# linum-uqam/ViT-OCM-WMSegmentation

Measured on AMD Instinct MI355X. Metric: OCM tiles/s (224x224, ViT-S/16 attention-map inference), higher is better.
Workload: dtype bf16x3

## Files before the change

vit-ocm-wmsegmentation_amd/csrc/dev_knobs.h:

```cpp
#pragma once
#ifdef OCM_DEV
extern int g_ocm_knobs[8];
#define OCM_KNOB(i) (g_ocm_knobs[(i)])
#else
#define OCM_KNOB(i) 0
#endif
```

vit-ocm-wmsegmentation_amd/csrc/engine.hip:

```cpp
#include <stdarg.h>
#include <stdio.h>
#include <string.h>

#include <atomic>
#include <mutex>
#include <string>
#include <vector>

#include "host_common.h"
#include "launch.h"
#include "dev_knobs.h"
#include "attn_plan.h"
#include "otsu.h"

static thread_local std::string g_err;

int ocm_fail(int code, const char *fmt, ...) {
    char buf[512];
    va_list ap;
    va_start(ap, fmt);
    vsnprintf(buf, sizeof buf, fmt, ap);
    va_end(ap);
    g_err = buf;
    return code;
}
#define fail ocm_fail

Prof g_prof;

extern "C" int ocm_prof_begin(uint32_t class_mask, int32_t max_launches) {
    std::lock_guard<std::mutex> lk(g_prof.mu);
    if (g_prof.on.load(std::memory_order_relaxed)) return fail(OCM_ESTATE, "profiling already active");
    if (max_launches <= 0) return fail(OCM_EINVAL, "max_launches must be positive");
    g_prof.ev.resize((size_t)max_launches * 2);
    g_prof.cls.assign(max_launches, 0);
    for (auto &e : g_prof.ev) HIP_TRY(hipEventCreate(&e));
    g_prof.used = 0;
    g_prof.mask = class_mask;
    ++g_prof.gen;
    g_prof.on.store(true, std::memory_order_release);
    return OCM_OK;
}

extern "C" int ocm_prof_end(double *ms_per_class, int64_t *launches_per_class) {
    std::lock_guard<std::mutex> lk(g_prof.mu);
    if (!g_prof.on.load(std::memory_order_relaxed)) return fail(OCM_ESTATE, "profiling is not active");
    g_prof.on.store(false, std::memory_order_release);
    for (int c = 0; c < OCM_K_COUNT; ++c) {
        if (ms_per_class) ms_per_class[c] = 0.0;
        if (launches_per_class) launches_per_class[c] = 0;
    }
    int rc = OCM_OK;
    for (size_t i = 0; i < g_prof.used; ++i) {
        float ms = 0.f;
        hipError_t e = hipEventSynchronize(g_prof.ev[2 * i + 1]);
        if (e == hipSuccess) e = hipEventElapsedTime(&ms, g_prof.ev[2 * i], g_prof.ev[2 * i + 1]);
        if (e != hipSuccess) {
            rc = fail(OCM_EHIP, "event timing failed: %s", hipGetErrorString(e));
            break;
        }
        if (ms_per_class) ms_per_class[g_prof.cls[i]] += ms;
        if (launches_per_class) launches_per_class[g_prof.cls[i]] += 1;
    }
    for (auto &e : g_prof.ev) (void)hipEventDestroy(e);
    g_prof.ev.clear();
    g_prof.cls.clear();
    g_prof.used = 0;
    return rc;
}

#ifdef OCM_DEV
extern "C" int ocm_debug_knob(int32_t which, int32_t value) {
    if (which < 0 || which >= 8) return fail(OCM_EINVAL, "knob %d out of range", which);
    g_ocm_knobs[which] = value;
    return OCM_OK;
}
#endif

extern "C" int ocm_abi_version(void) { return OCM_ABI_VERSION; }
extern "C" const char *ocm_last_error(void) { return g_err.c_str(); }
extern "C" int32_t ocm_n_pad(int32_t n_tokens) { return ocm_round_up(n_tokens, 8); }
extern "C" int32_t ocm_n_pad_prec(int32_t precision, int32_t n_tokens) { return ocm_n_pad_for(precision, n_tokens); }

enum ParamKind { P_F32, P_BF16, P_PATCH };
struct Param {
    std::string name;
    ParamKind kind;
    size_t count;
    size_t offset;
    bool set;
    bool optional = false;
};

struct BlockP {
    int ln1_g, ln1_b, qkv_w, qkv_b, proj_w, proj_b, ln2_g, ln2_b, fc1_w, fc1_b, fc2_w, fc2_b;
    int qkv_w32 = -1, fc1_w32 = -1, qkv_wf = -1, fc1_wf = -1, qkv_c = -1, qkv_d = -1, fc1_c = -1, fc1_d = -1;
    bool fold_dirty = true;
};

struct ocm_vit {
    ocm_vit_config cfg;
    int D, H, L, M, p, C, Kpe;
    int hd;
    bool mfma_heads() const { return hd == 64 || hd == 128; }
    int prec;
    size_t esz;
    std::vector<Param> params;
    std::vector<BlockP> blk;
    int cls, pe_w, pe_b, norm_g, norm_b, mask_tok;
    char *arena;
    size_t arena_bytes;
    hipGraphExec_t graph_exec = nullptr;
    hipStream_t graph_stream = nullptr;
    ocm_vit_io graph_key;
    bool graph_valid = false;
    uint64_t graph_hits = 0, graph_captures = 0;
    int32_t opt[OCM_OPT_COUNT] = {0};
    bool can_fold() const { return prec == 2; }
    bool folding() const { return can_fold() && opt[OCM_OPT_FOLD_LN] != 1; }

    int add(const std::string &name, ParamKind kind, size_t count, size_t stored_elems) {
        Param pr{name, kind, count, arena_bytes, false};
        const size_t bytes = stored_elems * (kind == P_F32 ? 4 : esz);
        arena_bytes += (bytes + 255) & ~(size_t)255;
        params.push_back(pr);
        return (int)params.size() - 1;
// ... 918 lines not shown
```

vit-ocm-wmsegmentation_amd/csrc/gemm_core.h:

```cpp
#pragma once
#include <type_traits>
#include "common.h"

#ifdef OCM_GEMM_STAMPS
__device__ unsigned long long g_wstamps[512 * 16 * 8];
#define WSTAMP(k)                                                                                       \
    do {                                                                                                \
        if (t == nsteps / 2 && (threadIdx.x & 63) == 0 && blockIdx.x < 512)                              \
            g_wstamps[(blockIdx.x * 16 + (threadIdx.x >> 6 & 15)) * 8 + (k)] = __builtin_readcyclecounter(); \
    } while (0)
__device__ unsigned long long g_stamps[8192 * 8];
#define STAMP(i)                                                                                        \
    do {                                                                                                \
        if (threadIdx.x == 0 && blockIdx.x < 8192) g_stamps[blockIdx.x * 8 + (i)] = __builtin_readcyclecounter(); \
    } while (0)
#else
#define STAMP(i) ((void)0)
#define WSTAMP(k) ((void)0)
#endif

template <int BM_, int BN_, int WAVES_M_, int WAVES_N_, int MF16_ = 0>
struct GemmCfg {
    static constexpr int BM = BM_, BN = BN_, WAVES_M = WAVES_M_, WAVES_N = WAVES_N_, MF16 = MF16_;
    static constexpr int NT = WAVES_M * WAVES_N * OCM_WAVE;
// ... 443 lines not shown
    int bc = 0, bi = D % NSTAGE;
#ifdef OCM_GEMM_STAMPS
    unsigned long long stamp_wait = 0;
#endif
    for (int t = 0; t < nsteps; ++t) {
        const int younger = min(D - 1, nsteps - 1 - t);
#ifdef OCM_GEMM_STAMPS
        const unsigned long long tw0 = __builtin_readcyclecounter();
#endif
        WSTAMP(0);
        wait_vm_steps<LPS, NSTAGE - 2>(younger);
        WSTAMP(1);
#ifdef OCM_GEMM_STAMPS
        const unsigned long long tw1 = __builtin_readcyclecounter();
#endif
        raw_barrier();
#ifdef OCM_GEMM_STAMPS
        if (t == 0) STAMP(6);
        if (t > 0) {
            const unsigned long long tw2 = __builtin_readcyclecounter();
            stamp_wait += ((tw2 - tw1) << 32) | ((tw1 - tw0) & 0xFFFFFFFFull);
        }
#endif
        WSTAMP(2);
#if !defined(OCM_ABL) || OCM_ABL != 2
        if (t + D < nsteps) OCM_DMA_ISSUE(t + D, bi);
#endif
        __builtin_amdgcn_sched_barrier(0);
        WSTAMP(3);
        compute(bc);
#ifdef OCM_GEMM_STAMPS
        if (t == nsteps / 2) {
            __builtin_amdgcn_sched_barrier(0);
            asm volatile("v_mov_b32 %0, %0\n\ts_nop 0" : "+v"(acc[TM - 1][TN - 1][15]));
            WSTAMP(4);
        }
#endif
        bc = bc + 1 == NSTAGE ? 0 : bc + 1;
        bi = bi + 1 == NSTAGE ? 0 : bi + 1;
    }
    raw_barrier();
#ifdef OCM_GEMM_STAMPS
    if (threadIdx.x == 0 && blockIdx.x < 8192) g_stamps[blockIdx.x * 8 + 7] = stamp_wait;
#endif
#undef OCM_DMA_ISSUE
}

constexpr int EPI_MAXS = 6;
struct EpiPre {
    f32x2 raw[EPI_MAXS];
    f32x2 cd;
};
struct EpiNoPre {};
template <class Cfg, class Epi>
__device__ __forceinline__ auto epi_prefetch(const Epi &epi, int m0, int n0, int M, int N) {
    if constexpr (Epi::ROWTAB) {
        EpiPre p;
#pragma unroll
        for (int i = 0; i < EPI_MAXS; ++i) p.raw[i] = f32x2{0.f, 0.f};
        p.cd = f32x2{0.f, 0.f};
        if (threadIdx.x < Cfg::BM) epi.row_raw(min(m0 + (int)threadIdx.x, M - 1), p.raw);
        if (threadIdx.x < Cfg::BN) p.cd = epi.col_entry(min(n0 + (int)threadIdx.x, N - 1));
        return p;
    } else {
        return EpiNoPre();
    }
}

template <class Cfg, bool SWAP, class Epi, int LDS_AVAIL = Cfg::LDS_BYTES, class Pre = EpiNoPre, int ACCL = 0>
__device__ __forceinline__ void run_epilogue(const f32x16 (&acc)[Cfg::TM][Cfg::TN], char *smem, const Epi &epi, int m0,
                                             int n0, bool active = true, const Pre *pre = nullptr) {
    f32x2 *rowtab = (f32x2 *)(smem + LDS_AVAIL), *coltab = rowtab + Cfg::BM;
    if constexpr (Epi::ROWTAB) {
        if (threadIdx.x < Cfg::BM) rowtab[threadIdx.x] = epi.row_final(pre->raw);
        if (threadIdx.x < Cfg::BN) coltab[threadIdx.x] = pre->cd;
    }
    const int lane = threadIdx.x & 63, wave = threadIdx.x >> 6;
    const int wm = wave / Cfg::WAVES_N, wn = wave % Cfg::WAVES_N;
    const int r = lane & 31, h = lane >> 5;
    if constexpr (Cfg::BM * Cfg::BN * 4 <= LDS_AVAIL) {
        constexpr int COLS = SWAP ? Cfg::BM : Cfg::BN;
        float *C = (float *)smem;
        if (active)
#pragma unroll
        for (int i = 0; i < Cfg::TM; ++i)
#pragma unroll
            for (int j = 0; j < Cfg::TN; ++j) {
                const bool half = Cfg::HALF && i == Cfg::TM - 1;
                const int tm = half ? (Cfg::TM - 1) * Cfg::RB + wm * 16 : (i * Cfg::WAVES_M + wm) * 32, tn = (j * Cfg::WAVES_N + wn) * 32;
                const int row0 = SWAP ? tn : tm, col0 = SWAP ? tm : tn;
#pragma unroll
                for (int e = 0; e < (half ? 8 : 16); ++e)
                    C[(row0 + acc_rpos<ACCL>(e, lane)) * COLS + col0 + acc_cpos<ACCL>(e, lane)] = acc[i][j][e];
            }
        STAMP(2);
        lds_barrier();
        STAMP(3);
        if (active) epi.template run<PassCfg<Cfg::BM, Cfg::BN, Cfg::NT>>((const float *)C, m0, n0, rowtab, coltab);
    } else if constexpr (!SWAP) {
        constexpr int PASS = Cfg::RB * Cfg::BN * 4;
        static_assert(PASS <= LDS_AVAIL, "a row band must fit the operand LDS");
        constexpr int NBUF = 2 * PASS <= LDS_AVAIL ? 2 : 1;
#pragma unroll
        for (int i = 0; i < Cfg::TM; ++i) {
            if (NBUF == 1 && i) lds_barrier();
            float *C = (float *)(smem + (i % NBUF) * PASS);
            const bool half = Cfg::HALF && i == Cfg::TM - 1;
            if (active)
#pragma unroll
            for (int j = 0; j < Cfg::TN; ++j) {
                const int col0 = (j * Cfg::WAVES_N + wn) * 32;
#pragma unroll
                for (int e = 0; e < (half ? 8 : 16); ++e)
                    C[(wm * (half ? 16 : 32) + acc_rpos<ACCL>(e, lane)) * Cfg::BN + col0 + acc_cpos<ACCL>(e, lane)] = acc[i][j][e];
            }
            lds_barrier();
            if (active) {
                if (half)
                    epi.template run<PassCfg<Cfg::RB / 2, Cfg::BN, Cfg::NT>>((const float *)C, m0 + i * Cfg::RB, n0, rowtab + i * Cfg::RB, coltab);
                else
                    epi.template run<PassCfg<Cfg::RB, Cfg::BN, Cfg::NT>>((const float *)C, m0 + i * Cfg::RB, n0, rowtab + i * Cfg::RB, coltab);
            }
        }
    } else {
        static_assert(!Cfg::HALF, "half tiles: normal orientation only");
        constexpr int PASS = Cfg::CB * Cfg::BM * 4;
        static_assert(PASS <= LDS_AVAIL, "a column band must fit the operand LDS");
        constexpr int NBUF = 2 * PASS <= LDS_AVAIL ? 2 : 1;
#pragma unroll
        for (int j = 0; j < Cfg::TN; ++j) {
            if (NBUF == 1 && j) lds_barrier();
            float *C = (float *)(smem + (j % NBUF) * PASS);
            if (active)
#pragma unroll
            for (int i = 0; i < Cfg::TM; ++i) {
                const int col0 = (i * Cfg::WAVES_M + wm) * 32;
#pragma unroll
                for (int e = 0; e < 16; ++e)
                    C[(wn * 32 + acc_rpos<ACCL>(e, lane)) * Cfg::BM + col0 + acc_cpos<ACCL>(e, lane)] = acc[i][j][e];
            }
            lds_barrier();
            if (active) epi.template run<PassCfg<Cfg::BM, Cfg::CB, Cfg::NT>>((const float *)C, m0, n0 + j * Cfg::CB, rowtab, coltab + j * Cfg::CB);
        }
    }
}

template <class Cfg, class E, bool SWAP, int KSTEPS, int NSTAGE, class Epi, int A_AUX = 0>
__global__ __launch_bounds__(Cfg::NT) void gemm_dma_kernel(const E *__restrict__ A, int64_t lda, const E *__restrict__ W,
                                                           int64_t ldw, int M, int N, int K, Epi epi) {
    extern __shared__ __attribute__((aligned(16))) char smem[];
    const int tiles_n = (N + Cfg::BN - 1) / Cfg::BN;
    const int id = xcd_remap(blockIdx.x, gridDim.x);
    const int tm = id / tiles_n, tn = id - tm * tiles_n;
    const int m0 = tm * Cfg::BM, n0 = tn * Cfg::BN;
    f32x16 acc[Cfg::TM][Cfg::TN];
    const auto pre = epi_prefetch<Cfg>(epi, m0, n0, M, N);
    STAMP(0);
#if defined(OCM_ABL) && OCM_ABL == 4
#pragma unroll
    for (int i = 0; i < Cfg::TM; ++i)
#pragma unroll
        for (int j = 0; j < Cfg::TN; ++j)
#pragma unroll
            for (int e = 0; e < 16; ++e) acc[i][j][e] = (float)(threadIdx.x + e);
#else
    gemm_mainloop_dma<Cfg, E, SWAP, KSTEPS, NSTAGE, A_AUX>(A, lda, W, ldw, m0, n0, M, N, K, smem, acc, epi.bias);
#endif
    STAMP(1);
#if defined(OCM_ABL) && OCM_ABL == 3
#pragma unroll
    for (int i = 0; i < Cfg::TM; ++i)
#pragma unroll
        for (int j = 0; j < Cfg::TN; ++j) asm volatile("" ::"v"(acc[i][j]));
#else
    run_epilogue<Cfg, SWAP, Epi, NSTAGE * (Cfg::BM + Cfg::BN) * 128, decltype(pre), accl_of<Cfg, E>()>(acc, smem, epi, m0, n0, true, &pre);
#endif
    STAMP(4);
#ifdef OCM_GEMM_STAMPS
    __builtin_amdgcn_s_waitcnt(0);
    STAMP(5);
#endif
}

template <class Cfg, class E, bool SWAP, int KSTEPS, class ALoad, class Epi>
__global__ __launch_bounds__(Cfg::NT) void gemm_kernel(ALoad al, const E *__restrict__ W, int64_t ldw, int M, int N,
                                                       int K, Epi epi) {
    extern __shared__ __attribute__((aligned(16))) char smem[];
    const int tiles_n = (N + Cfg::BN - 1) / Cfg::BN;
    const int id = xcd_remap(blockIdx.x, gridDim.x);
    const int tm = id / tiles_n, tn = id - tm * tiles_n;
    const int m0 = tm * Cfg::BM, n0 = tn * Cfg::BN;
    f32x16 acc[Cfg::TM][Cfg::TN];
    const auto pre = epi_prefetch<Cfg>(epi, m0, n0, M, N);
    STAMP(0);
    gemm_mainloop<Cfg, E, SWAP, KSTEPS>(al, W, ldw, m0, n0, M, N, K, smem, acc, epi.bias);
    STAMP(1);
    run_epilogue<Cfg, SWAP, Epi, Cfg::LDS_BYTES, decltype(pre), accl_of<Cfg, E>()>(acc, smem, epi, m0, n0, true, &pre);
    STAMP(4);
#ifdef OCM_GEMM_STAMPS
    __builtin_amdgcn_s_waitcnt(0);
    STAMP(5);
#endif
}
```

vit-ocm-wmsegmentation_amd/csrc/gemm_kernels.h:

```cpp
#pragma once
#include <type_traits>
#include "gemm_core.h"
#include "launch.h"
#include "gemm_plan.h"
#include "dev_knobs.h"

int ocm_wt_mask();

template <GemmTile T>
using CfgOf = GemmCfg<GEMM_TILES[T].bm, GEMM_TILES[T].bn, GEMM_TILES[T].waves_m, GEMM_TILES[T].waves_n, GEMM_TILES[T].mf16>;
typedef CfgOf<T128x128> Cfg128x128;
typedef CfgOf<T128x128q> Cfg128x128q;
typedef CfgOf<T128x128q16> Cfg128x128q16;
typedef CfgOf<T128x128m16> Cfg128x128m16;
typedef CfgOf<T160x128q16> Cfg160x128q16;
typedef CfgOf<T256x256m16> Cfg256x256m16;
typedef CfgOf<T64x128> Cfg64x128;
typedef CfgOf<T64x128w> Cfg64x128w;
typedef CfgOf<T64x64> Cfg64x64;
typedef CfgOf<T256x256> Cfg256x256;
typedef CfgOf<T256x128> Cfg256x128;
typedef CfgOf<T128x192> Cfg128x192;
typedef CfgOf<T128x96> Cfg128x96;

// ... 94 lines not shown
            const int q = threadIdx.x + i * NT, row = q / CPR, col = (q - row * CPR) * W;
            const int m = m0 + row, n = n0 + col;
            if ((TOTAL % NT != 0 && q >= TOTAL) || m >= M || n >= N) continue;
            const int64_t o = (int64_t)m * ldo + n;
            f32x4 v0 = *(const f32x4 *)(C + row * BN + col);
            if (!ACT_OUT) {
                if (MODE == 1) v0 += rs[i];
                if (MODE == 4) {
#pragma unroll
                    for (int e = 0; e < 4; ++e) v0[e] = fmaxf(v0[e], 0.f);
                }
                *(f32x4 *)((float *)out + o) = v0;
            } else {
                f32x4 v1 = v0;
                if (W == 8) v1 = *(const f32x4 *)(C + row * BN + col + 4);
                if (ln.stats) {
                    const f32x2 mr = rowtab[row];
                    const float mu = mr[0], rstd = mr[1];
#pragma unroll
                    for (int e = 0; e < 4; ++e) {
                        const f32x2 cd = coltab[col + e];
                        v0[e] = fmaf(rstd, fmaf(-mu, cd[0], v0[e]), cd[1]);
                    }
                    if (W == 8) {
#pragma unroll
                        for (int e = 0; e < 4; ++e) {
                            const f32x2 cd = coltab[col + 4 + e];
                            v1[e] = fmaf(rstd, fmaf(-mu, cd[0], v1[e]), cd[1]);
                        }
                    }
                }
                if (MODE == 2) {
#pragma unroll
                    for (int e = 0; e < 4; e += 2) {
                        const f32x2 a = gelu_erf2(f32x2{v0[e], v0[e + 1]});
                        v0[e] = a[0];
                        v0[e + 1] = a[1];
                        if (W == 8) {
                            const f32x2 b = gelu_erf2(f32x2{v1[e], v1[e + 1]});
                            v1[e] = b[0];
                            v1[e + 1] = b[1];
                        }
                    }
                }
                if (wt)
                    store_act_wt((OE *)nullptr, (char *)out + (int64_t)m * ldo * (int)sizeof(OE), n, v0, v1);
                else
                    store_act((OE *)nullptr, (char *)out + (int64_t)m * ldo * (int)sizeof(OE), n, v0, v1);
            }
        }
    }
};

template <class OE>
struct EpiResidStats {
    static constexpr bool ROWTAB = false;
    static constexpr int BN_MULT = 64;
    const float *bias;
    const float *resid;
    float *x;
    void *xs;
    float *stats;
    int M, N;
    int wt = 3;
    float *shift = nullptr;
    const float *prev_stats = nullptr, *prev_shift = nullptr;
    __device__ __forceinline__ static void st16(void *p, const f32x4 &v, bool through) {
        if (through)
            asm volatile("global_store_dwordx4 %0, %1, off sc1\n\ts_nop 1" ::"v"(p), "v"(v) : "memory");
        else
            *(f32x4 *)p = v;
    }
    template <class Cfg>
    __device__ __forceinline__ void run(const float *C, int m0, int n0, const f32x2 *, const f32x2 *) const {
        constexpr int BM = Cfg::BM, BN = Cfg::BN, NT = Cfg::NT, NV = BN / 64, RPP = NT / 8;
        static_assert(BN % 64 == 0 && NT % 64 == 0, "eight lanes x eight columns per chunk");
        const int sub = threadIdx.x & 7, grp = threadIdx.x >> 3;
        constexpr int NPASS = (BM + RPP - 1) / RPP, NPRE = NPASS <= 2 ? NPASS : 1;
        f32x4 pre[NPRE][NV][2];
#pragma unroll
        for (int ps = 0; ps < NPRE; ++ps) {
            const int64_t mo = (int64_t)min(m0 + ps * RPP + grp, M - 1) * N;
#pragma unroll
            for (int i = 0; i < NV; ++i) {
                pre[ps][i][0] = *(const f32x4 *)(resid + mo + n0 + sub * 8 + i * 64);
                pre[ps][i][1] = *(const f32x4 *)(resid + mo + n0 + sub * 8 + i * 64 + 4);
            }
        }
#pragma unroll 2
        for (int r0 = 0; r0 < BM; r0 += RPP) {
            const int row = r0 + grp, m = m0 + row;
            const bool ok = row < BM && m < M;
            const int64_t mo = (int64_t)min(m, M - 1) * N;
            f32x4 v[NV][2];
#pragma unroll
            for (int i = 0; i < NV; ++i) {
                if (NPRE == NPASS) {
                    v[i][0] = pre[NPASS == 2 && r0 ? 1 : 0][i][0];
                    v[i][1] = pre[NPASS == 2 && r0 ? 1 : 0][i][1];
                } else {
                    v[i][0] = *(const f32x4 *)(resid + mo + n0 + sub * 8 + i * 64);
                    v[i][1] = *(const f32x4 *)(resid + mo + n0 + sub * 8 + i * 64 + 4);
                }
            }
            float sh = 0.f;
            if (shift) {
                const int nslot = N >> 6;
                float ps = 0.f;
                if (prev_stats)
                    for (int i = sub; i < nslot; i += 8) ps += prev_stats[((int64_t)min(m, M - 1) * nslot + i) * 2];
#pragma unroll
                for (int o = 4; o > 0; o >>= 1) ps += __shfl_xor(ps, o, 64);
                sh = (prev_shift ? prev_shift[min(m, M - 1)] : 0.f) + ps / (float)N;
                if (ok && n0 == 0 && sub == 0) shift[m] = sh;
            }
            float s1 = 0.f, s2 = 0.f;
            char *rowp = (char *)xs + mo * (int)sizeof(OE);
#pragma unroll
            for (int i = 0; i < NV; ++i) {
                const int n = n0 + sub * 8 + i * 64;
                const float *cp = C + min(row, BM - 1) * BN + sub * 8 + i * 64;
                v[i][0] += *(const f32x4 *)cp;
                v[i][1] += *(const f32x4 *)(cp + 4);
                if (ok) {
                    st16(x + mo + n, v[i][0], wt & 1);
                    st16(x + mo + n + 4, v[i][1], wt & 1);
                }
                v[i][0] -= sh;
                v[i][1] -= sh;
                if (ok) {
                    if constexpr (Elem<OE>::MODE == 2) {
                        bf16x8 hi, lo;
                        split8(v[i][0], v[i][1], hi, lo);
                        st16(rowp + sp_off(n), __builtin_bit_cast(f32x4, hi), wt & 2);
                        st16(rowp + sp_off(n) + 64, __builtin_bit_cast(f32x4, lo), wt & 2);
                    } else if constexpr (Elem<OE>::MODE == 1) {
                        *(f32x4 *)(rowp + n * 4) = v[i][0];
                        *(f32x4 *)(rowp + n * 4 + 16) = v[i][1];
                    } else {
                        *(bf16x8 *)(rowp + n * 2) = cvt8(v[i][0], v[i][1]);
                    }
                }
#pragma unroll
                for (int e = 0; e < 4; ++e) {
                    s1 += v[i][0][e] + v[i][1][e];
                    s2 = fmaf(v[i][0][e], v[i][0][e], fmaf(v[i][1][e], v[i][1][e], s2));
                }
            }
#pragma unroll
            for (int o = 4; o > 0; o >>= 1) {
                s1 += __shfl_xor(s1, o, 64);
                s2 += __shfl_xor(s2, o, 64);
            }
            if (ok && sub < NV) {
                const f32x2 val = {sub ? 0.f : s1, sub ? 0.f : s2};
                *((f32x2 *)stats + (int64_t)m * (N >> 6) + (n0 >> 6) + sub) = val;
            }
        }
    }
};

template <class Cfg, class E, bool SWAP, int KSTEPS, class ALoad, class Epi>
static hipError_t launch_gemm_ks(const ALoad &al, const E *w, int64_t ldw, int M, int N, int K, const Epi &epi,
                                 hipStream_t s) {
    auto kern = gemm_kernel<Cfg, E, SWAP, KSTEPS, ALoad, Epi>;
    constexpr int LDS = Cfg::LDS_BYTES + (Epi::ROWTAB ? (Cfg::BM + Cfg::BN) * 8 : 0);
// ... 127 lines not shown
                                hipStream_t s) {
    EpiLinear<4, E> epi{bias, nullptr, out, M, N, ldo};
    return launch_linear_epi<4, E>(a, w, epi, M, N, K, s);
}

template <class Cfg, class E, int KSTEPS, int NSTAGE>
__global__ __launch_bounds__(Cfg::NT) void gemm_dma_splitk_kernel(const E *__restrict__ A, int64_t lda,
                                                                  const E *__restrict__ W, int64_t ldw, int M, int N,
                                                                  int Kslice, float *__restrict__ part) {
    extern __shared__ __attribute__((aligned(16))) char smem[];
    const int tiles_n = (N + Cfg::BN - 1) / Cfg::BN;
    const int tm = blockIdx.x / tiles_n, tn = blockIdx.x - tm * tiles_n, slice = blockIdx.y;
    const int m0 = tm * Cfg::BM, n0 = tn * Cfg::BN;
    EpiLinear<0, E> epi{nullptr, nullptr, part + (size_t)slice * M * N, M, N, N};
    f32x16 acc[Cfg::TM][Cfg::TN];
    const auto pre = epi_prefetch<Cfg>(epi, m0, n0, M, N);
    gemm_mainloop_dma<Cfg, E, false, KSTEPS, NSTAGE>(A + (size_t)slice * Kslice, lda, W + (size_t)slice * Kslice, ldw, m0, n0, M,
                                                     N, Kslice, smem, acc, (const float *)nullptr);
    run_epilogue<Cfg, false, EpiLinear<0, E>, NSTAGE * (Cfg::BM + Cfg::BN) * 128, decltype(pre), accl_of<Cfg, E>()>(acc, smem, epi, m0, n0, true,
                                                                                                  &pre);
}

template <class E>
static hipError_t launch_linear_splitk(const E *a, const E *w, const float *bias, const float *resid, float *x, int M, int N,
                                       int K, hipStream_t s, const StatsOut &so) {
    typedef Cfg64x64 Cfg;
    constexpr int NSTAGE = 4, KS = OCM_SPLITK_STEPS;
    constexpr int LDS = NSTAGE * (Cfg::BM + Cfg::BN) * 128;
    auto kern = gemm_dma_splitk_kernel<Cfg, E, KS, NSTAGE>;
    static OptinMask optin;
    if (hipError_t e = lds_optin((const void *)kern, LDS, optin); e != hipSuccess) return e;
    const int tiles = ((M + Cfg::BM - 1) / Cfg::BM) * (N / Cfg::BN);
    kern<<<dim3(tiles, OCM_SPLITK), dim3(Cfg::NT), LDS, s>>>(a, K, w, K, M, N, K / OCM_SPLITK, so.part);
    if (hipError_t e = hipGetLastError(); e != hipSuccess) return e;
    return launch_splitk_finish(so.part, OCM_SPLITK, bias, resid, x, so.xs, so.stats, M, N, s, so);
}

template <class E>
hipError_t launch_linear_e(const E *a, const E *w, const float *bias, const float *resid, void *out, int M, int N,
                                  int K, int epilogue, hipStream_t s, const LnFold &ln, const StatsOut &so) {
    switch (epilogue) {
        case 0: return launch_linear_mode<0, E>(a, w, bias, resid, out, M, N, K, s);
        case 1:
            if constexpr (Elem<E>::MODE == 2)
                if (so.part && resid && (!so.stats || so.xs) && K % Elem<E>::KROW == 0) {
                    const GemmPlan p = gemm_plan_linear(2, 1, M, N, K, so.stats != nullptr, true, OCM_KNOB(0));
                    if (p.splitk > 1) return launch_linear_splitk<E>(a, w, bias, resid, (float *)out, M, N, K, s, so);
                }
            if (so.stats) {
                if (N % 64) return hipErrorInvalidValue;
                EpiResidStats<E> epi{bias, resid, (float *)out, so.xs, so.stats, M, N};
                epi.shift = so.shift, epi.prev_stats = so.prev_stats, epi.prev_shift = so.prev_shift;
                epi.wt = OCM_KNOB(5) ? OCM_KNOB(5) - 1 : 0;
                return launch_linear_epi<1, E>(a, w, epi, M, N, K, s);
            }
            return launch_linear_mode<1, E>(a, w, bias, resid, out, M, N, K, s);
        case 2: return launch_linear_mode<2, E>(a, w, bias, resid, out, M, N, K, s, ln);
        case 3: return launch_linear_mode<3, E>(a, w, bias, resid, out, M, N, K, s, ln);
    }
    return hipErrorInvalidValue;
}

template <int MODE, class E>
static hipError_t launch_linear_ld_mode(const E *a, int64_t lda, const E *w, const float *bias, const float *resid,
                                        void *out, int64_t ldo, int M, int N, int K, hipStream_t s) {
    if (K % Elem<E>::KROW) return hipErrorInvalidValue;
    RowLoader<E> al{a, lda};
    EpiLinear<MODE, E> epi{bias, resid, out, M, N, ldo};
    const GemmPlan p = gemm_plan_linear_ld(Elem<E>::MODE, M, N, K);
    switch (p.tile) {
        case T128x128: return launch_gemm<Cfg128x128, E, false>(al, w, K, M, N, K, epi, s, p.ksteps);
        case T64x128: return launch_gemm<Cfg64x128, E, false>(al, w, K, M, N, K, epi, s, p.ksteps);
        case T64x64: return launch_gemm<Cfg64x64, E, false>(al, w, K, M, N, K, epi, s, p.ksteps);
        default: return hipErrorInvalidValue;
    }
}

template <class E>
hipError_t launch_linear_ld_e(const E *a, int64_t lda, const E *w, const float *bias, const float *resid, void *out,
                                     int64_t ldo, int M, int N, int K, int epilogue, hipStream_t s) {
    switch (epilogue) {
        case 0: return launch_linear_ld_mode<0, E>(a, lda, w, bias, resid, out, ldo, M, N, K, s);
        case 1: return launch_linear_ld_mode<1, E>(a, lda, w, bias, resid, out, ldo, M, N, K, s);
        case 2: return launch_linear_ld_mode<2, E>(a, lda, w, bias, resid, out, ldo, M, N, K, s);
        case 3: return launch_linear_ld_mode<3, E>(a, lda, w, bias, resid, out, ldo, M, N, K, s);
    }
    return hipErrorInvalidValue;
}

template <class OE, int D_>
struct EpiResidLN {
    static constexpr bool ROWTAB = false;
    const float *bias;
    const float *resid;
    float *x;
    const float *gamma, *beta;
    void *xn;
    int M;
    float eps;
    int wt = 0;
    template <class Cfg>
    __device__ __forceinline__ void run(const float *C, int m0, int, const f32x2 *, const f32x2 *) const {
        constexpr int BM = Cfg::BM, NT = Cfg::NT, NV = D_ / 128;
        static_assert(Cfg::BN == D_ && D_ % 128 == 0, "full rows, float4 lanes");
        const int sub = threadIdx.x & 31, half = threadIdx.x >> 5;
        constexpr int RPP = NT / 32;
// ... 559 lines not shown
```

vit-ocm-wmsegmentation_amd/csrc/kernels_attn.hip:

```cpp
#include <stdlib.h>

#include "launch.h"

#define LOG2E 1.4426950408889634f
int ocm_wt_mask();
#include "dev_knobs.h"
#include "attn_plan.h"
#define OCM_VMCNT_ATTN(n) asm volatile("s_waitcnt vmcnt(%0)" ::"n"(n) : "memory")

#ifndef OCM_DEFER_MAX
#define OCM_DEFER_MAX 8.0f
#endif
__device__ __forceinline__ float defer_max_update(float &m, float cand) {
    if (__any(cand > m + OCM_DEFER_MAX)) {
        const float mn = fmaxf(m, cand);
        const float alpha = fast_exp2(m - mn);
        m = mn;
        return alpha;
    }
    return 1.0f;
}

template <bool WANT_O, int HD = 64>
__global__ __launch_bounds__(256, HD == 64 ? 3 : 2) void attn_fwd_kernel(const bf16 *__restrict__ Q, const bf16 *__restrict__ Kk,
// ... 777 lines not shown
    if (!active) return;
    const float lt = l + __shfl_xor(l, 32, 64);
    const int qrow = q0 + r;
    if (KSPLIT) {
        if (qrow < N) {
            float *dst = part + (((int64_t)blockIdx.z * gridDim.y + bh) * N + qrow) * (HD + 4);
            if (h == 0) *(f32x2 *)(dst + HD) = f32x2{m, lt};
            if (WANT_O) {
#pragma unroll
                for (int db = 0; db < ND; ++db)
#pragma unroll
                    for (int g = 0; g < 4; ++g) {
                        f32x4 o;
#pragma unroll
                        for (int e = 0; e < 4; ++e) o[e] = O[db][4 * g + e];
                        *(f32x4 *)(dst + 32 * db + 8 * g + 4 * h) = o;
                    }
            }
        }
        return;
    }
    if (qrow < N) {
        if (lse2 && h == 0) lse2[(int64_t)bh * N + qrow] = m + __log2f(lt);
        if (WANT_O) {
            const float inv = 1.0f / lt;
            const int b = bh / H, head = bh - b * H;
            char *dst = ctx + ((int64_t)b * N + qrow) * (H * HD) * 4 + head * (HD * 4);
#pragma unroll
            for (int db = 0; db < ND; ++db)
#pragma unroll
                for (int g = 0; g < 4; ++g) {
                    f32x4 o;
#pragma unroll
                    for (int e = 0; e < 4; ++e) o[e] = O[db][4 * g + e] * inv;
                    bf16x4 oh, ol;
                    split4(o, oh, ol);
                    char *p = dst + db * 128 + (8 * g + 4 * h) * 2;
                    if (wt) {
                        const f32x2 dh = __builtin_bit_cast(f32x2, oh), dl = __builtin_bit_cast(f32x2, ol);
                        asm volatile("global_store_dwordx2 %0, %1, off sc1\n\ts_nop 1" ::"v"(p), "v"(dh) : "memory");
                        asm volatile("global_store_dwordx2 %0, %1, off sc1\n\ts_nop 1" ::"v"(p + 64), "v"(dl) : "memory");
                    } else {
                        *(bf16x4 *)p = oh;
                        *(bf16x4 *)(p + 64) = ol;
                    }
                }
        }
    }
    ASTAMP(15);
    ASTAMP_RT(13);
}


template <bool WANT_O>
__global__ __launch_bounds__(256, 3) void attn_fwd_x3_pp_kernel(const char *__restrict__ Q, const char *__restrict__ Kk,
                                                               const char *__restrict__ Vt, char *__restrict__ ctx,
                                                               float *__restrict__ lse2, int N, int npad, int H, float scale2) {
    constexpr int NW = 4, HD = 64, KB = HD * 128, KP = 8 / NW, VP = WANT_O ? 8 / NW : 0;
    __shared__ __attribute__((aligned(1024))) char smem[6 * KB];
    const int tid = threadIdx.x, lane = tid & 63;
    const int wave = __builtin_amdgcn_readfirstlane(tid >> 6);
    const int r = lane & 31, h = lane >> 5;
    int qblk, bh;
    xcd_remap2(qblk, bh);
    const int q0 = (qblk * NW + wave) * 32;
    const bool active = q0 < N;
    const char *Qb = Q + (int64_t)bh * npad * (HD * 4);
    const char *Kb = Kk + (int64_t)bh * npad * (HD * 4);
    const char *Vb = Vt + (int64_t)bh * HD * npad * 4;
    const int nt = (N + 31) >> 5;

    bf16x8 qh[4], ql[4];
    x3_load_q(Qb + (int64_t)min(q0 + r, N - 1) * (HD * 4), h, qh, ql);
    int voffK[KP], voffV[VP ? VP : 1];
    x3_piece_offsets<HD, NW, KP, VP>(lane, wave, npad, voffK, voffV);
#if defined(__HIP_DEVICE_COMPILE__)
    const auto rsK = x3_tile_rsrc<HD>(Kb, npad), rsV = x3_tile_rsrc<HD>(Vb, npad);
#define OCM_PP_DMA_K(t, slot)                                                                                        \
    do {                                                                                                             \
        _Pragma("unroll") for (int j = 0; j < KP; ++j)                                                               \
            __builtin_amdgcn_raw_ptr_buffer_load_lds(rsK, (lds_ptr)(smem + (slot) * KB + (j * NW + wave) * 1024), 16, \
                                                     voffK[j], (t) * (32 * HD * 4), 0, 0);                           \
    } while (0)
#define OCM_PP_DMA_V(t, slot)                                                                                              \
    do {                                                                                                                   \
        _Pragma("unroll") for (int j = 0; j < VP; ++j)                                                                     \
            __builtin_amdgcn_raw_ptr_buffer_load_lds(rsV, (lds_ptr)(smem + (3 + (slot)) * KB + (j * NW + wave) * 1024), 16, \
                                                     voffV[j], (t) * 128, 0, 0);                                           \
    } while (0)
#else
#define OCM_PP_DMA_K(t, slot) (void)0
#define OCM_PP_DMA_V(t, slot) (void)0
#endif
    OCM_PP_DMA_K(0, 0);
    if (nt > 1) OCM_PP_DMA_K(1, 1);
    if (WANT_O) OCM_PP_DMA_V(0, 0);
    if (nt > 2) OCM_PP_DMA_K(2, 2);
    if (WANT_O && nt > 1) OCM_PP_DMA_V(1, 1);
    __builtin_amdgcn_s_waitcnt(0x0F70);
    auto block_barrier = [&]() {
        __builtin_amdgcn_sched_barrier(0);
        asm volatile("s_waitcnt lgkmcnt(0)" ::: "memory");
        __builtin_amdgcn_s_barrier();
        asm volatile("" ::: "memory");
        __builtin_amdgcn_sched_barrier(0);
    };
    block_barrier();

    f32x16 O[2], S;
    bf16x8 ph[2], pl[2];
#pragma unroll
    for (int e = 0; e < 16; ++e) O[0][e] = O[1][e] = S[e] = 0.f;
#pragma unroll
    for (int s2 = 0; s2 < 2; ++s2)
#pragma unroll
        for (int e = 0; e < 8; ++e) ph[s2][e] = pl[s2][e] = (bf16)0.f;
    float m = -INFINITY, l = 0.f;
    const int pr = pi_row(r);
    const int first_pad = N - (nt - 1) * 32;

    auto qk = [&](int ks) {
        const char *Kt = smem + ks * KB;
#pragma unroll
        for (int e = 0; e < 16; ++e) S[e] = 0.f;
#pragma unroll
        for (int s = 0; s < 4; ++s) {
            const char *kp = Kt + (s >> 1) * 4096;
            const bf16x8 kh = *(const bf16x8 *)(kp + lds_off(pr, (s & 1) * 2 + h));
            const bf16x8 kl = *(const bf16x8 *)(kp + lds_off(pr, 4 + (s & 1) * 2 + h));
            S = mfma32x3(kh, kl, qh[s], ql[s], S);
        }
    };
    auto Mblk = [&](int vs, int ks, bool more) {
        if (WANT_O) {
            const char *Vtile = smem + (3 + vs) * KB;
#pragma unroll
            for (int s2 = 0; s2 < 2; ++s2)
#pragma unroll
                for (int db = 0; db < 2; ++db) {
                    const char *vp = Vtile + db * 32 * 128;
                    const bf16x8 vh = *(const bf16x8 *)(vp + lds_off(r, 2 * s2 + h));
                    const bf16x8 vl = *(const bf16x8 *)(vp + lds_off(r, 4 + 2 * s2 + h));
                    O[db] = mfma32x3(vh, vl, ph[s2], pl[s2], O[db]);
                }
        }
        if (more) qk(ks);
    };
    auto Vblk = [&](bool last_of_seq) {
        if (last_of_seq && first_pad < 32) x3_mask_pad_keys(S, first_pad, h);
        const float alpha = x3_softmax(S, scale2, m, l);
        if (WANT_O) {
            x3_rescale(O, alpha);
#pragma unroll
            for (int s2 = 0; s2 < 2; ++s2) x3_split_p(S, s2, ph[s2], pl[s2]);
        }
    };

    if (active) {
        qk(0);
        Vblk(nt == 1);
    }
    block_barrier();

    int s0 = 0, s1 = 1;
    for (int kt = 0; kt < nt; ++kt) {
        const int s2n = s1 == 2 ? 0 : s1 + 1;
        if (kt + 3 < nt) OCM_PP_DMA_K(kt + 3, s0);
        if (WANT_O && kt + 2 < nt) OCM_PP_DMA_V(kt + 2, s2n);
        const bool last = kt + 1 == nt;
        if (WANT_O && last && first_pad < 32) {
            x3_zero_pad_keys<HD, 64>(smem + (3 + s0) * KB, tid >> 2, tid & 3, first_pad);
            block_barrier();
        }
        if (active) {
            Mblk(s0, s1, !last);
            if (!last) Vblk(kt + 2 == nt);
        }
        if (kt + 3 < nt)
            OCM_VMCNT_ATTN(KP + VP);
        else if (WANT_O && kt + 2 < nt)
            OCM_VMCNT_ATTN(VP);
        else
            OCM_VMCNT_ATTN(0);
        block_barrier();
        s0 = s1;
        s1 = s2n;
    }
#undef OCM_PP_DMA_K
#undef OCM_PP_DMA_V

    if (!active) return;
    const float lt = l + __shfl_xor(l, 32, 64);
    const int qrow = q0 + r;
    if (lse2 && h == 0 && qrow < N) lse2[(int64_t)bh * N + qrow] = m + __log2f(lt);
    if (WANT_O) {
        const float inv = 1.0f / lt;
        const int b = bh / H, head = bh - b * H;
        char *dst = ctx + ((int64_t)b * N + min(qrow, N - 1)) * (H * HD) * 4 + head * (HD * 4);
#pragma unroll
        for (int db = 0; db < 2; ++db)
#pragma unroll
            for (int g = 0; g < 4; g += 2) {
                f32x4 oa, ob;
#pragma unroll
                for (int e = 0; e < 4; ++e) {
                    oa[e] = O[db][4 * g + e] * inv;
                    ob[e] = O[db][4 * g + 4 + e] * inv;
                }
                bf16x4 ah, al, bhh, bl;
                split4(oa, ah, al);
                split4(ob, bhh, bl);
                uint2 ahu = __builtin_bit_cast(uint2, ah), alu = __builtin_bit_cast(uint2, al);
                uint2 bhu = __builtin_bit_cast(uint2, bhh), blu = __builtin_bit_cast(uint2, bl);
                auto sw = [](unsigned &x, unsigned &y) {
// ... 475 lines not shown
    }
    attn_generic_kernel<<<dim3((nq + 3) / 4, batch * heads), dim3(256), lds, s>>>(
        qkv, (char *)ctx, attn, query_rows, n_rows, rows, batch, heads, n_tokens, head_dim, scale, prec, all);
    return hipGetLastError();
}

size_t attention_ksplit_bytes(int prec, int batch, int n_tokens, int heads, int head_dim) {
    return attn_plan_workspace_bytes(prec, batch, n_tokens, heads, head_dim);
}

hipError_t launch_attention(int prec, const void *q, const void *k, const void *vt, void *ctx, float *lse2, int batch,
                            int n_tokens, int n_pad, int heads, float scale, hipStream_t s, int head_dim, float *ksplit_ws,
                            size_t ksplit_bytes) {
    if (head_dim != 64 && head_dim != 128) return hipErrorInvalidValue;
    if (prec == 2 && n_pad % 32) return hipErrorInvalidValue;
    const AttnPlan p = attn_plan(prec, batch, n_tokens, heads, head_dim, ksplit_ws ? ksplit_bytes : 0, OCM_KNOB(6), OCM_KNOB(7));
    const dim3 grid(p.grid_x, p.grid_y, p.grid_z), block(p.waves * 64);
    const float scale2 = scale * LOG2E;
    const char *Q = (const char *)q, *K = (const char *)k, *V = (const char *)vt;
    switch (p.kernel) {
        case ATTN_BF16_WHOLE: {
            auto kern = ctx ? attn_small_kernel<true> : attn_small_kernel<false>;
            kern<<<grid, block, 0, s>>>((const bf16 *)q, (const bf16 *)k, (const bf16 *)vt, (bf16 *)ctx, lse2, n_tokens, n_pad, heads,
                                        scale2);
            break;
        }
        case ATTN_BF16_STREAM: {
            auto kern = head_dim == 128 ? (ctx ? attn_fwd_kernel<true, 128> : attn_fwd_kernel<false, 128>)
                                        : (ctx ? attn_fwd_kernel<true> : attn_fwd_kernel<false>);
            kern<<<grid, block, 0, s>>>((const bf16 *)q, (const bf16 *)k, (const bf16 *)vt, (bf16 *)ctx, lse2, n_tokens, n_pad, heads,
                                        scale2);
            break;
        }
        case ATTN_F32_STREAM: {
            auto kern = head_dim == 128 ? (ctx ? attn_fwd_f32_kernel<true, 128> : attn_fwd_f32_kernel<false, 128>)
                                        : (ctx ? attn_fwd_f32_kernel<true> : attn_fwd_f32_kernel<false>);
            if (p.lds_bytes > 64 * 1024) {
                static OptinMask optin[2];
                if (hipError_t e = lds_optin((const void *)kern, p.lds_bytes, optin[ctx ? 1 : 0]); e != hipSuccess) return e;
            }
            kern<<<grid, block, p.lds_bytes, s>>>((const float *)q, (const float *)k, (const float *)vt, (float *)ctx, lse2, n_tokens,
                                                  n_pad, heads, scale2);
            break;
        }
        case ATTN_X3_WS: {
            auto kern = ctx ? attn_fwd_x3_ws_kernel<true> : attn_fwd_x3_ws_kernel<false>;
            static OptinMask optin[2];
            if (hipError_t e = lds_optin((const void *)kern, p.lds_bytes, optin[ctx ? 1 : 0]); e != hipSuccess) return e;
            kern<<<grid, block, p.lds_bytes, s>>>(Q, K, V, (char *)ctx, lse2, n_tokens, n_pad, heads, scale2);
            break;
        }
        case ATTN_X3_PP: {
            auto kern = ctx ? attn_fwd_x3_pp_kernel<true> : attn_fwd_x3_pp_kernel<false>;
            kern<<<grid, block, 0, s>>>(Q, K, V, (char *)ctx, lse2, n_tokens, n_pad, heads, scale2);
            break;
        }
        case ATTN_X3_DMA:
            if (head_dim == 128) {
                auto kern = ctx ? attn_fwd_x3_dma_kernel<true, 4, 2, 128, 2> : attn_fwd_x3_dma_kernel<false, 4, 2, 128, 2>;
                kern<<<grid, block, 0, s>>>(Q, K, V, (char *)ctx, lse2, n_tokens, n_pad, heads, scale2, 0, nullptr);
            } else {
                auto kern = ctx ? attn_fwd_x3_dma_kernel<true, 8, 2> : attn_fwd_x3_dma_kernel<false, 8, 2>;
                kern<<<grid, block, 0, s>>>(Q, K, V, (char *)ctx, lse2, n_tokens, n_pad, heads, scale2, (ocm_wt_mask() >> 4) & 1,
                                            nullptr);
            }
            break;
        case ATTN_X3_DMA_KSPLIT: {
            auto kern = ctx ? attn_fwd_x3_dma_kernel<true, 8, 2, 64, 3, true> : attn_fwd_x3_dma_kernel<false, 8, 2, 64, 3, true>;
            kern<<<grid, block, 0, s>>>(Q, K, V, (char *)ctx, lse2, n_tokens, n_pad, heads, scale2, 0, ksplit_ws);
            if (hipError_t e = hipGetLastError(); e != hipSuccess) return e;
            const int64_t rows = (int64_t)batch * heads * n_tokens;
            attn_merge_x3_kernel<64><<<dim3((unsigned)((rows + 15) / 16)), dim3(256), 0, s>>>(
                ksplit_ws, p.kslices, (char *)ctx, lse2, batch * heads, n_tokens, heads);
            break;
        }
    }
    return hipGetLastError();
}

template <int HD>
static hipError_t launch_probs_hd(int prec, const void *q, const void *k, const float *lse2, float *attn, int n_tokens, int n_pad,
                                  float scale2, dim3 grid, dim3 gridz, hipStream_t s) {
    const dim3 block(256);
    if (prec == 2)
        attn_probs_x3_kernel<HD><<<gridz, block, 0, s>>>((const char *)q, (const char *)k, lse2, attn, n_tokens, n_pad, scale2);
    else if (prec)
        attn_probs_f32_kernel<HD><<<grid, block, 0, s>>>((const float *)q, (const float *)k, lse2, attn, n_tokens, n_pad, scale2);
    else
        attn_probs_kernel<HD><<<grid, block, 0, s>>>((const bf16 *)q, (const bf16 *)k, lse2, attn, n_tokens, n_pad, scale2);
    return hipGetLastError();
}

hipError_t launch_attention_probs(int prec, const void *q, const void *k, const float *lse2, float *attn, int batch,
                                  int n_tokens, int n_pad, int heads, float scale, hipStream_t s, int head_dim,
                                  const int32_t *query_rows, int n_rows, float *rows) {
    if (head_dim != 64 && head_dim != 128) return hipErrorInvalidValue;
    const int qtiles = (n_tokens + 31) / 32;
    const dim3 grid((qtiles + 3) / 4, batch * heads);
    const int wgs = (int)(grid.x * grid.y), ktiles = qtiles;
    int nz = wgs >= 256 ? 1 : min(ktiles, min(16, (512 + wgs - 1) / wgs));
    if (OCM_KNOB(2) > 0) nz = min(ktiles, OCM_KNOB(2));
    const dim3 gridz(grid.x, grid.y, nz);
    if (n_rows <= 0) rows = nullptr;
    bool folded = false;
    hipError_t e;
    if (prec == 2 && head_dim == 64 && n_tokens <= 255 && n_pad % 32 == 0 && n_pad >= n_tokens) {
// ... 153 lines not shown
```

vit-ocm-wmsegmentation_amd/csrc/kernels_gemm.hip:

```cpp
#include "launch.h"
#include "host_common.h"
#include "dev_knobs.h"

template <class E>
hipError_t launch_linear_e(const E *a, const E *w, const float *bias, const float *resid, void *out, int M, int N, int K,
                           int epilogue, hipStream_t s, const LnFold &ln, const StatsOut &so);
template <class E>
hipError_t launch_linear_ld_e(const E *a, int64_t lda, const E *w, const float *bias, const float *resid, void *out,
                              int64_t ldo, int M, int N, int K, int epilogue, hipStream_t s);
template <class E>
hipError_t launch_resid_ln_e(const E *a, const E *w, const float *bias, const float *resid, float *x, const float *gamma,
                             const float *beta, void *xn, int M, int D, int K, float eps, hipStream_t s);
template <class E>
hipError_t launch_qkv_e(const E *a, const E *w, const float *bias, E *q, E *k, E *vt, float *qkv_f32, int batch,
                        int n_tokens, int n_pad, int heads, int head_dim, bool want_v, hipStream_t s, const LnFold &ln);
template <class E>
hipError_t launch_patch_e(const PatchArgs &pa, const E *w, const float *bias, const float *pos, float *x, int dim,
                          hipStream_t s, const StatsOut &so);

#ifdef OCM_DEV
int g_ocm_knobs[8] = {0, 0, 0, 0, 0, 0, 0, 0};
#endif
int ocm_wt_mask() { return OCM_KNOB(1) == 0 ? 35 : OCM_KNOB(1) < 0 ? 0 : OCM_KNOB(1); }

hipError_t launch_linear_ld(int prec, const void *a, int64_t lda, const void *w, const float *bias, const float *resid,
                            void *out, int64_t ldo, int M, int N, int K, int epilogue, hipStream_t s) {
    if (prec == 2) return hipErrorInvalidValue;
    if (prec)
        return launch_linear_ld_e<float>((const float *)a, lda, (const float *)w, bias, resid, out, ldo, M, N, K, epilogue,
                                         s);
    return launch_linear_ld_e<bf16>((const bf16 *)a, lda, (const bf16 *)w, bias, resid, out, ldo, M, N, K, epilogue, s);
}

hipError_t launch_linear(int prec, const void *a, const void *w, const float *bias, const float *resid, void *out, int M,
                         int N, int K, int epilogue, hipStream_t s, const LnFold &ln, const StatsOut &so) {
    if (prec == 2) return launch_linear_e<sp32>((const sp32 *)a, (const sp32 *)w, bias, resid, out, M, N, K, epilogue, s, ln, so);
    if (prec) return launch_linear_e<float>((const float *)a, (const float *)w, bias, resid, out, M, N, K, epilogue, s, ln, so);
    return launch_linear_e<bf16>((const bf16 *)a, (const bf16 *)w, bias, resid, out, M, N, K, epilogue, s, ln, so);
}

bool linear_resid_ln_supported(int D) { return D == 128 || D == 256 || D == 384; }

hipError_t launch_linear_resid_ln(int prec, const void *a, const void *w, const float *bias, const float *resid, float *x,
                                  const float *gamma, const float *beta, void *xn, int M, int D, int K, float eps,
                                  hipStream_t s) {
    if (prec == 2)
        return launch_resid_ln_e<sp32>((const sp32 *)a, (const sp32 *)w, bias, resid, x, gamma, beta, xn, M, D, K, eps, s);
    if (prec)
        return launch_resid_ln_e<float>((const float *)a, (const float *)w, bias, resid, x, gamma, beta, xn, M, D, K, eps, s);
    return launch_resid_ln_e<bf16>((const bf16 *)a, (const bf16 *)w, bias, resid, x, gamma, beta, xn, M, D, K, eps, s);
}

hipError_t launch_qkv(int prec, const void *a, const void *w, const float *bias, void *q, void *k, void *vt,
                      float *qkv_f32, int batch, int n_tokens, int n_pad, int heads, int head_dim, bool want_v,
                      hipStream_t s, const LnFold &ln) {
    if (prec == 2)
        return launch_qkv_e<sp32>((const sp32 *)a, (const sp32 *)w, bias, (sp32 *)q, (sp32 *)k, (sp32 *)vt, qkv_f32, batch,
                                  n_tokens, n_pad, heads, head_dim, want_v, s, ln);
    if (prec)
        return launch_qkv_e<float>((const float *)a, (const float *)w, bias, (float *)q, (float *)k, (float *)vt, qkv_f32,
                                   batch, n_tokens, n_pad, heads, head_dim, want_v, s, ln);
    return launch_qkv_e<bf16>((const bf16 *)a, (const bf16 *)w, bias, (bf16 *)q, (bf16 *)k, (bf16 *)vt, qkv_f32, batch,
                              n_tokens, n_pad, heads, head_dim, want_v, s, ln);
}

hipError_t launch_patch_embed(int prec, const PatchArgs &pa, const void *w, const float *bias, const float *pos,
                              float *x, int dim, hipStream_t s, const StatsOut &so) {
    if (prec == 2) return launch_patch_e<sp32>(pa, (const sp32 *)w, bias, pos, x, dim, s, so);
    if (prec) return launch_patch_e<float>(pa, (const float *)w, bias, pos, x, dim, s, so);
    return launch_patch_e<bf16>(pa, (const bf16 *)w, bias, pos, x, dim, s, so);
}

extern "C" int ocm_gemm_plan(int32_t family, int32_t precision, int32_t epilogue, int32_t M, int32_t N, int32_t K,
                             uint32_t flags, ocm_gemm_plan_info *plan) {
// ... 40 lines not shown
```

Before: 28620.

## Prefetch residual-stats epilogue inputs before mainloop and relax attention prologue waits

The residual-statistics GEMM epilogue now loads the previous-layer stats and shift values into registers before the main loop, so their latency overlaps the GEMM instead of stalling the epilogue. Separately, the bf16x3 ping-pong attention kernel always issues its K/V prologue DMAs (clamped to the last tile) and waits with a partial vmcnt instead of draining all loads, so it can start computing earlier. Dev knobs 8 and 9 restore the old behaviour for comparison. The cost is extra register pressure during the GEMM main loop and some redundant DMA traffic when there are few tiles.

```diff
diff --git a/vit-ocm-wmsegmentation_amd/csrc/dev_knobs.h b/vit-ocm-wmsegmentation_amd/csrc/dev_knobs.h
--- a/vit-ocm-wmsegmentation_amd/csrc/dev_knobs.h
+++ b/vit-ocm-wmsegmentation_amd/csrc/dev_knobs.h
@@ -1,6 +1,6 @@
 #pragma once
 #ifdef OCM_DEV
-extern int g_ocm_knobs[8];
+extern int g_ocm_knobs[10];
 #define OCM_KNOB(i) (g_ocm_knobs[(i)])
 #else
 #define OCM_KNOB(i) 0
diff --git a/vit-ocm-wmsegmentation_amd/csrc/engine.hip b/vit-ocm-wmsegmentation_amd/csrc/engine.hip
--- a/vit-ocm-wmsegmentation_amd/csrc/engine.hip
+++ b/vit-ocm-wmsegmentation_amd/csrc/engine.hip
@@ -71,7 +71,7 @@
 
 #ifdef OCM_DEV
 extern "C" int ocm_debug_knob(int32_t which, int32_t value) {
-    if (which < 0 || which >= 8) return fail(OCM_EINVAL, "knob %d out of range", which);
+    if (which < 0 || which >= 10) return fail(OCM_EINVAL, "knob %d out of range", which);
     g_ocm_knobs[which] = value;
     return OCM_OK;
 }
diff --git a/vit-ocm-wmsegmentation_amd/csrc/gemm_core.h b/vit-ocm-wmsegmentation_amd/csrc/gemm_core.h
--- a/vit-ocm-wmsegmentation_amd/csrc/gemm_core.h
+++ b/vit-ocm-wmsegmentation_amd/csrc/gemm_core.h
@@ -519,6 +519,18 @@
     f32x2 cd;
 };
 struct EpiNoPre {};
+
+template <class Epi, class Cfg, bool WHOLE, class = void>
+struct epi_own_pre {
+    static constexpr bool v = false;
+    typedef EpiNoPre type;
+};
+template <class Epi, class Cfg, bool WHOLE>
+struct epi_own_pre<Epi, Cfg, WHOLE, std::void_t<typename Epi::template Pre<Cfg, WHOLE>>> {
+    static constexpr bool v = true;
+    typedef typename Epi::template Pre<Cfg, WHOLE> type;
+};
+
 template <class Cfg, class Epi>
 __device__ __forceinline__ auto epi_prefetch(const Epi &epi, int m0, int n0, int M, int N) {
     if constexpr (Epi::ROWTAB) {
@@ -563,7 +575,12 @@
         STAMP(2);
         lds_barrier();
         STAMP(3);
-        if (active) epi.template run<PassCfg<Cfg::BM, Cfg::BN, Cfg::NT>>((const float *)C, m0, n0, rowtab, coltab);
+        if (active) {
+            if constexpr (epi_own_pre<Epi, Cfg, true>::v && std::is_same<Pre, typename epi_own_pre<Epi, Cfg, true>::type>::value)
+                epi.template run<PassCfg<Cfg::BM, Cfg::BN, Cfg::NT>>((const float *)C, m0, n0, rowtab, coltab, pre);
+            else
+                epi.template run<PassCfg<Cfg::BM, Cfg::BN, Cfg::NT>>((const float *)C, m0, n0, rowtab, coltab);
+        }
     } else if constexpr (!SWAP) {
         constexpr int PASS = Cfg::RB * Cfg::BN * 4;
         static_assert(PASS <= LDS_AVAIL, "a row band must fit the operand LDS");
@@ -621,6 +638,24 @@
     const int tm = id / tiles_n, tn = id - tm * tiles_n;
     const int m0 = tm * Cfg::BM, n0 = tn * Cfg::BN;
     f32x16 acc[Cfg::TM][Cfg::TN];
+    constexpr int RING = NSTAGE * (Cfg::BM + Cfg::BN) * 128;
+#ifndef OCM_ABL
+    if constexpr (epi_own_pre<Epi, Cfg, (Cfg::BM * Cfg::BN * 4 <= RING)>::v && !SWAP) {
+        typedef typename epi_own_pre<Epi, Cfg, (Cfg::BM * Cfg::BN * 4 <= RING)>::type OwnPre;
+        OwnPre pre;
+        epi.prefetch(pre, m0, n0);
+        STAMP(0);
+        gemm_mainloop_dma<Cfg, E, SWAP, KSTEPS, NSTAGE, A_AUX>(A, lda, W, ldw, m0, n0, M, N, K, smem, acc, epi.bias);
+        STAMP(1);
+        run_epilogue<Cfg, SWAP, Epi, RING, OwnPre, accl_of<Cfg, E>()>(acc, smem, epi, m0, n0, true, &pre);
+        STAMP(4);
+#ifdef OCM_GEMM_STAMPS
+        __builtin_amdgcn_s_waitcnt(0);
+        STAMP(5);
+#endif
+        return;
+    }
+#endif
     const auto pre = epi_prefetch<Cfg>(epi, m0, n0, M, N);
     STAMP(0);
 #if defined(OCM_ABL) && OCM_ABL == 4
diff --git a/vit-ocm-wmsegmentation_amd/csrc/gemm_kernels.h b/vit-ocm-wmsegmentation_amd/csrc/gemm_kernels.h
--- a/vit-ocm-wmsegmentation_amd/csrc/gemm_kernels.h
+++ b/vit-ocm-wmsegmentation_amd/csrc/gemm_kernels.h
@@ -170,7 +170,7 @@
     }
 };
 
-template <class OE>
+template <class OE, bool EARLY = true>
 struct EpiResidStats {
     static constexpr bool ROWTAB = false;
     static constexpr int BN_MULT = 64;
@@ -189,12 +189,39 @@
         else
             *(f32x4 *)p = v;
     }
+    template <class Cfg, bool WHOLE>
+    struct Pre {
+        static constexpr int RPP = Cfg::NT / 8, NPASS = (Cfg::BM + RPP - 1) / RPP;
+        static constexpr bool ON = EARLY && WHOLE && NPASS <= 2;
+        static constexpr int LSLOT = 2;
+        float st[ON ? NPASS : 1][LSLOT];
+        float psh[ON ? NPASS : 1];
+    };
+    template <class P>
+    __device__ __forceinline__ void prefetch(P &p, int m0, int n0) const {
+        if constexpr (P::ON) {
+            const int sub = threadIdx.x & 7, grp = threadIdx.x >> 3, nslot = N >> 6;
+#pragma unroll
+            for (int ps = 0; ps < P::NPASS; ++ps) {
+                const int64_t mc = min(m0 + ps * P::RPP + grp, M - 1);
+#pragma unroll
+                for (int k = 0; k < P::LSLOT; ++k)
+                    p.st[ps][k] = shift && prev_stats ? prev_stats[(mc * nslot + min(sub + 8 * k, nslot - 1)) * 2] : 0.f;
+                p.psh[ps] = shift && prev_shift ? prev_shift[mc] : 0.f;
+            }
+        }
+    }
     template <class Cfg>
-    __device__ __forceinline__ void run(const float *C, int m0, int n0, const f32x2 *, const f32x2 *) const {
+    __device__ __forceinline__ void run(const float *C, int m0, int n0, const f32x2 *rowtab, const f32x2 *coltab) const {
+        run<Cfg>(C, m0, n0, rowtab, coltab, (const Pre<Cfg, false> *)nullptr);
+    }
+    template <class Cfg, class P>
+    __device__ __forceinline__ void run(const float *C, int m0, int n0, const f32x2 *, const f32x2 *, const P *early) const {
         constexpr int BM = Cfg::BM, BN = Cfg::BN, NT = Cfg::NT, NV = BN / 64, RPP = NT / 8;
         static_assert(BN % 64 == 0 && NT % 64 == 0, "eight lanes x eight columns per chunk");
         const int sub = threadIdx.x & 7, grp = threadIdx.x >> 3;
         constexpr int NPASS = (BM + RPP - 1) / RPP, NPRE = NPASS <= 2 ? NPASS : 1;
+        static_assert(!P::ON || (P::NPASS == NPASS && P::RPP == RPP), "the prefetch was laid out for this tile");
         f32x4 pre[NPRE][NV][2];
 #pragma unroll
         for (int ps = 0; ps < NPRE; ++ps) {
@@ -210,12 +237,13 @@
             const int row = r0 + grp, m = m0 + row;
             const bool ok = row < BM && m < M;
             const int64_t mo = (int64_t)min(m, M - 1) * N;
+            const int pass = NPASS == 2 && r0 ? 1 : 0;
             f32x4 v[NV][2];
 #pragma unroll
             for (int i = 0; i < NV; ++i) {
                 if (NPRE == NPASS) {
-                    v[i][0] = pre[NPASS == 2 && r0 ? 1 : 0][i][0];
-                    v[i][1] = pre[NPASS == 2 && r0 ? 1 : 0][i][1];
+                    v[i][0] = pre[pass][i][0];
+                    v[i][1] = pre[pass][i][1];
                 } else {
                     v[i][0] = *(const f32x4 *)(resid + mo + n0 + sub * 8 + i * 64);
                     v[i][1] = *(const f32x4 *)(resid + mo + n0 + sub * 8 + i * 64 + 4);
@@ -225,11 +253,28 @@
             if (shift) {
                 const int nslot = N >> 6;
                 float ps = 0.f;
-                if (prev_stats)
+                bool summed = false;
+                if constexpr (P::ON) {
+                    if (prev_stats && nslot <= 8 * P::LSLOT) {
+#pragma unroll
+                        for (int k = 0; k < P::LSLOT; ++k) {
+                            float slot = early->st[pass][k];
+                            asm volatile("" : "+v"(slot));
+                            if (sub + 8 * k < nslot) ps += slot;
+                        }
+                        summed = true;
+                    }
+                }
+                if (prev_stats && !summed)
                     for (int i = sub; i < nslot; i += 8) ps += prev_stats[((int64_t)min(m, M - 1) * nslot + i) * 2];
 #pragma unroll
                 for (int o = 4; o > 0; o >>= 1) ps += __shfl_xor(ps, o, 64);
-                sh = (prev_shift ? prev_shift[min(m, M - 1)] : 0.f) + ps / (float)N;
+                float psh = 0.f;
+                if constexpr (P::ON)
+                    psh = early->psh[pass];
+                else
+                    psh = prev_shift ? prev_shift[min(m, M - 1)] : 0.f;
+                sh = psh + ps / (float)N;
                 if (ok && n0 == 0 && sub == 0) shift[m] = sh;
             }
             float s1 = 0.f, s2 = 0.f;
@@ -463,6 +508,14 @@
                 EpiResidStats<E> epi{bias, resid, (float *)out, so.xs, so.stats, M, N};
                 epi.shift = so.shift, epi.prev_stats = so.prev_stats, epi.prev_shift = so.prev_shift;
                 epi.wt = OCM_KNOB(5) ? OCM_KNOB(5) - 1 : 0;
+#ifdef OCM_DEV
+                if (OCM_KNOB(8) == 1) {
+                    EpiResidStats<E, false> late{bias, resid, (float *)out, so.xs, so.stats, M, N};
+                    late.shift = so.shift, late.prev_stats = so.prev_stats, late.prev_shift = so.prev_shift;
+                    late.wt = epi.wt;
+                    return launch_linear_epi<1, E>(a, w, late, M, N, K, s);
+                }
+#endif
                 return launch_linear_epi<1, E>(a, w, epi, M, N, K, s);
             }
             return launch_linear_mode<1, E>(a, w, bias, resid, out, M, N, K, s);
diff --git a/vit-ocm-wmsegmentation_amd/csrc/kernels_attn.hip b/vit-ocm-wmsegmentation_amd/csrc/kernels_attn.hip
--- a/vit-ocm-wmsegmentation_amd/csrc/kernels_attn.hip
+++ b/vit-ocm-wmsegmentation_amd/csrc/kernels_attn.hip
@@ -853,7 +853,7 @@
 }
 
 
-template <bool WANT_O>
+template <bool WANT_O, bool WAIT_ALL = false>
 __global__ __launch_bounds__(256, 3) void attn_fwd_x3_pp_kernel(const char *__restrict__ Q, const char *__restrict__ Kk,
                                                                const char *__restrict__ Vt, char *__restrict__ ctx,
                                                                float *__restrict__ lse2, int N, int npad, int H, float scale2) {
@@ -894,11 +894,12 @@
 #define OCM_PP_DMA_V(t, slot) (void)0
 #endif
     OCM_PP_DMA_K(0, 0);
-    if (nt > 1) OCM_PP_DMA_K(1, 1);
+    if (!WAIT_ALL || nt > 1) OCM_PP_DMA_K(min(1, nt - 1), 1);
     if (WANT_O) OCM_PP_DMA_V(0, 0);
-    if (nt > 2) OCM_PP_DMA_K(2, 2);
-    if (WANT_O && nt > 1) OCM_PP_DMA_V(1, 1);
-    __builtin_amdgcn_s_waitcnt(0x0F70);
+    if (!WAIT_ALL || nt > 2) OCM_PP_DMA_K(min(2, nt - 1), 2);
+    if (WANT_O && (!WAIT_ALL || nt > 1)) OCM_PP_DMA_V(min(1, nt - 1), 1);
+    __builtin_amdgcn_s_waitcnt(0x0F70 | (WAIT_ALL ? 0 : 2 * KP + 2 * VP));
+    static_assert(2 * KP + 2 * VP < 16, "the count sits in the low four bits");
     auto block_barrier = [&]() {
         __builtin_amdgcn_sched_barrier(0);
         asm volatile("s_waitcnt lgkmcnt(0)" ::: "memory");
@@ -961,6 +962,7 @@
         qk(0);
         Vblk(nt == 1);
     }
+    if (!WAIT_ALL) OCM_VMCNT_ATTN(KP + VP);
     block_barrier();
 
     int s0 = 0, s1 = 1;
@@ -1542,6 +1544,9 @@
         }
         case ATTN_X3_PP: {
             auto kern = ctx ? attn_fwd_x3_pp_kernel<true> : attn_fwd_x3_pp_kernel<false>;
+#ifdef OCM_DEV
+            if (OCM_KNOB(9) == 1) kern = ctx ? attn_fwd_x3_pp_kernel<true, true> : attn_fwd_x3_pp_kernel<false, true>;
+#endif
             kern<<<grid, block, 0, s>>>(Q, K, V, (char *)ctx, lse2, n_tokens, n_pad, heads, scale2);
             break;
         }
diff --git a/vit-ocm-wmsegmentation_amd/csrc/kernels_gemm.hip b/vit-ocm-wmsegmentation_amd/csrc/kernels_gemm.hip
--- a/vit-ocm-wmsegmentation_amd/csrc/kernels_gemm.hip
+++ b/vit-ocm-wmsegmentation_amd/csrc/kernels_gemm.hip
@@ -19,7 +19,7 @@
                           hipStream_t s, const StatsOut &so);
 
 #ifdef OCM_DEV
-int g_ocm_knobs[8] = {0, 0, 0, 0, 0, 0, 0, 0};
+int g_ocm_knobs[10] = {0, 0, 0, 0, 0, 0, 0, 0, 0, 0};
 #endif
 int ocm_wt_mask() { return OCM_KNOB(1) == 0 ? 35 : OCM_KNOB(1) < 0 ? 0 : OCM_KNOB(1); }
 
```

Result: no change. 28710, median of 6 (+0.3%).
